# AIML-IfI/openset-imagenet

Hardware: AMD Instinct MI355X
Metric: images/sec (whole node) ResNet-50 + entropic-open-set, Protocol 2, 1/2/4/8 GPUs (higher is better)
Workload: dtype f32; 1 GPU; Protocol 2, ResNet-50, entropic open-set loss, batch 128/GPU; workload_key=p2, classes=30, batch_per_gpu=128, global_batch=128, image=3x224x224, loss=entropic, optimizer=adam lr=1e-3, parallelism=dp1

## Files before the change

openset-imagenet_amd/csrc/conv_wino.hip:

```cpp
#include "conv_common.h"
#include <algorithm>
#include <type_traits>
#include <utility>

using namespace osi_conv;

namespace {

#ifndef OSI_WABL
#define OSI_WABL 0
#endif
#ifndef OSI_FABL
#define OSI_FABL 0
#endif
#ifndef OSI_STAGE_OUT
#define OSI_STAGE_OUT 1
#endif
#ifndef OSI_XSPREAD
#define OSI_XSPREAD 8
#endif
constexpr int KC = 16;
constexpr int PF = 6;

struct WinoP {
// ... 236 lines not shown
#pragma unroll
        for (int j = 0; j < 2; ++j) {
            const int yy = 2 * th + i, xx = 2 * tw + j;
            const bool ok = live && t < p.T && yy < p.H && xx < p.W;
            po[i * 2 + j] = ok ? (uint32_t)((((b * p.H + yy) * p.W + xx) * p.Nc + (WIDE ? 128 : 64) * nt + 32 * wm + 4 * hh) * 4) : OOB;
        }
}

template <bool XF, int EPI, bool ODD, bool WIDE>
__global__ __launch_bounds__(256, 1) void k_wino(WinoP p) {
    constexpr int TB = WIDE ? 32 : 64, CW = WIDE ? 128 : 64, NV = WIDE ? 2 : 4;
    __shared__ __attribute__((aligned(16))) float sV[2 * 16 * TB * KC + (WIDE ? 16384 : 0)];
    __shared__ uint32_t sPo[256];
    const int tid = threadIdx.x, lane = tid & 63, wave = tid >> 6, wm = WIDE ? wave : wave >> 1, wn = WIDE ? 0 : wave & 1;
    const __amdgpu_buffer_rsrc_t rx = make_rsrc(p.x, p.x_bytes);
    const __amdgpu_buffer_rsrc_t ry = make_rsrc(p.y, p.y_bytes);
    const __amdgpu_buffer_rsrc_t ru = make_rsrc(p.u, p.u_bytes);
    const int G = gridDim.x, wg = blockIdx.x;
    const int ltile = WIDE ? tid >> 3 : tid >> 2, q = WIDE ? tid & 7 : tid & 3;
    const int ntile = 32 * wn + (lane & 31), hh = lane >> 5;
    const int THW = p.TH * p.TW;

    Seg seg = seg_first(wg, p.nfull, p.q, p.r, p.KS, G);
    if (!seg.valid) return;
    int mt, nt;
    unit_of(seg.v, p.MT, p.NT, mt, nt);

    uint32_t off[16];
    unsigned long long okm[16];
    uint32_t po[4], po_next[4];
    uint32_t ua, ua_next;
    auto setup = [&](int mt_, int nt_, bool live, uint32_t (&po_)[4], uint32_t& ua_) {
        {
            const int t = mt_ * TB + ltile;
            const int b = t / THW, rem = t - b * THW, th = rem / p.TW, tw = rem - th * p.TW;
            const uint32_t base = (uint32_t)((((b * p.H + 2 * th - 1) * p.W + 2 * tw - 1) * p.Kc + q * NV) * 4);
#pragma unroll
            for (int i = 0; i < 4; ++i)
#pragma unroll
                for (int j = 0; j < 4; ++j) {
                    const int yy = 2 * th - 1 + i, xx = 2 * tw - 1 + j;
                    const bool ok = live && t < p.T && (unsigned)yy < (unsigned)p.H && (unsigned)xx < (unsigned)p.W;
                    off[i * 4 + j] = ok ? base + (uint32_t)((i * p.W + j) * p.Kc * 4) : OOB;
                    if constexpr (XF) okm[i * 4 + j] = __builtin_amdgcn_ballot_w64(ok);
                }
        }
        out_offsets<WIDE>(p, mt_, nt_, ntile, wm, hh, live, po_);
        ua_ = (uint32_t)((((CW / 32) * nt_ + wm) * 2 * 64 + lane) * 16);
    };
    setup(mt, nt, true, po, ua);
    float* const wbase = sV + ltile * KC + (WIDE ? 4 * ((q >> 1) ^ ((ltile >> 2) & 3)) + 2 * (q & 1) : 4 * (q ^ ((ltile >> 2) & 3)));
    const float* const rb0 = sV + ntile * KC + 4 * ((0 + hh) ^ ((ntile >> 2) & 3));
    const float* const rb1 = sV + ntile * KC + 4 * ((2 + hh) ^ ((ntile >> 2) & 3));
    const uint32_t ustep = (uint32_t)p.CB * 2048;

    f32x16 acc[16];
    using XT = std::conditional_t<WIDE, f32x2, f32x4>;
    XT xr[16];
    auto load_x1 = [&](int ks, int k) {
        if constexpr (WIDE) xr[k] = __builtin_bit_cast(f32x2, __builtin_amdgcn_raw_buffer_load_b64(rx, off[k], (uint32_t)ks * (KC * 4), 0));
        else xr[k] = bld4(rx, off[k], (uint32_t)ks * (KC * 4));
    };
    auto load_x = [&](int ks) {
#pragma unroll
        for (int k = 0; k < 16; ++k) load_x1(ks, k);
    };
    auto act_col = [&](int j, const f32x4& sc4, const f32x4& sh4) {
        if constexpr (XF) {
#pragma unroll
            for (int i = 0; i < 4; ++i)
#pragma unroll
                for (int e = 0; e < NV; ++e)
                    asm volatile("v_fma_f32 %0, %0, %1, %2\n\tv_max_f32 %0, 0, %0\n\tv_cndmask_b32 %0, 0, %0, %3"
                                 : "+v"(xr[i * 4 + j][e]) : "v"(sc4[e]), "v"(sh4[e]), "s"(okm[i * 4 + j]));
        }
        {
            const XT d0 = xr[j], d1 = xr[4 + j], d2 = xr[8 + j], d3 = xr[12 + j];
            xr[j] = pk_sub(d0, d2); xr[4 + j] = pk_add(d1, d2); xr[8 + j] = pk_sub(d2, d1); xr[12 + j] = pk_sub(d1, d3);
        }
    };
    auto row_store = [&](int i, int buf) {
        float* w = wbase + buf * (16 * TB * KC) + (i * 4) * (TB * KC);
        const XT t0 = xr[i * 4], t1 = xr[i * 4 + 1], t2 = xr[i * 4 + 2], t3 = xr[i * 4 + 3];
        const XT o[4] = {pk_sub(t0, t2), pk_add(t1, t2), pk_sub(t2, t1), pk_sub(t1, t3)};
#pragma unroll
        for (int nu = 0; nu < 4; ++nu) *reinterpret_cast<XT*>(w + nu * (TB * KC)) = o[nu];
    };
    auto ld_scale = [&](int ks, f32x4& sc4, f32x4& sh4) {
        if constexpr (XF) {
            if constexpr (WIDE) {
                const f32x2 a = *reinterpret_cast<const f32x2*>(p.sc + ks * KC + 2 * q), b = *reinterpret_cast<const f32x2*>(p.sh + ks * KC + 2 * q);
                sc4[0] = a[0]; sc4[1] = a[1]; sh4[0] = b[0]; sh4[1] = b[1];
            } else {
                sc4 = ld4(p.sc + ks * KC + 4 * q);
                sh4 = ld4(p.sh + ks * KC + 4 * q);
            }
        }
    };

    f32x4 sc4 = {1, 1, 1, 1}, sh4 = {0, 0, 0, 0};
    load_x(seg.ks0);
    ld_scale(seg.ks0, sc4, sh4);
#pragma unroll
    for (int j = 0; j < 4; ++j) act_col(j, sc4, sh4);
#pragma unroll
    for (int i = 0; i < 4; ++i) row_store(i, 0);

    f32x4 a[16][2];
    auto load_u = [&](int pos, uint32_t base, int ks) {
        const uint32_t soff = (OSI_FABL & 1) ? 0u : (uint32_t)(pos * p.KS + ks) * ustep;
        a[pos][0] = bld4(ru, base, soff);
        a[pos][1] = bld4(ru, base + 1024u, soff);
    };
#pragma unroll
    for (int i = 0; i < PF; ++i) load_u(i, ua, seg.ks0);
    __syncthreads();

    int buf = 0;
    for (;;) {
#pragma unroll
        for (int i = 0; i < 16; ++i)
#pragma unroll
            for (int r = 0; r < 16; ++r) acc[i][r] = 0.f;
        Seg nxt{0, 0, 0, -1, false};
        const int cur_mt = mt, cur_nt = nt;
        for (int ks = seg.ks0; ks < seg.ks1; ++ks) {
            const bool last = ks + 1 == seg.ks1;
            int ksn = ks + 1;
            uint32_t uan = ua;
            if (last) {
                nxt = seg_next(seg, wg, p.nfull, p.q, p.r, p.KS, G);
                if (nxt.valid) unit_of(nxt.v, p.MT, p.NT, mt, nt);
                setup(mt, nt, nxt.valid, po_next, ua_next);
                ksn = nxt.valid ? nxt.ks0 : 0;
                uan = nxt.valid ? ua_next : ua;
            }
#if !(OSI_FABL & 2) && !OSI_XSPREAD
            load_x(ksn);
#endif
            ld_scale(ksn, sc4, sh4);
            const float* r0 = rb0 + buf * (16 * TB * KC);
            const float* r1 = rb1 + buf * (16 * TB * KC);
            f32x4 b0 = *reinterpret_cast<const f32x4*>(r0), b1 = *reinterpret_cast<const f32x4*>(r1);
            __builtin_amdgcn_sched_barrier(0);
            auto position = [&](auto POSC) {
                constexpr int pos = decltype(POSC)::value;
                if (pos + PF < 16) load_u(pos + PF, ua, ks);
                else load_u(pos + PF - 16, uan, ksn);
#if OSI_XSPREAD && !(OSI_FABL & 2)
                if constexpr (pos < OSI_XSPREAD) {
                    constexpr int n0 = pos * 16 / OSI_XSPREAD, n1 = (pos + 1) * 16 / OSI_XSPREAD;
#pragma unroll
                    for (int k = n0; k < n1; ++k) load_x1(ksn, k);
                }
#endif
                f32x4 nb0 = b0, nb1 = b1;
                if (pos < 15 && !(OSI_FABL & 8)) {
                    nb0 = *reinterpret_cast<const f32x4*>(r0 + (pos + 1) * (TB * KC));
                    nb1 = *reinterpret_cast<const f32x4*>(r1 + (pos + 1) * (TB * KC));
                }
                const f32x4 a0 = a[pos][0], a1 = a[pos][1];
#pragma unroll
                for (int e = 0; e < 4; ++e) acc[pos] = __builtin_amdgcn_mfma_f32_32x32x2f32(a0[e], b0[e], acc[pos], 0, 0, 0);
#pragma unroll
                for (int e = 0; e < 4; ++e) acc[pos] = __builtin_amdgcn_mfma_f32_32x32x2f32(a1[e], b1[e], acc[pos], 0, 0, 0);
#if !(OSI_FABL & 4)
                if constexpr (pos >= 8 && pos < 12) act_col(pos - 8, sc4, sh4);
                if constexpr (pos >= 12) row_store(pos - 12, buf ^ 1);
#endif
                b0 = nb0; b1 = nb1;
                __builtin_amdgcn_sched_barrier(0);
            };
            for_each_const(position, std::make_integer_sequence<int, 16>{});
            __syncthreads();
            buf ^= 1;
        }

        const int ch0 = CW * cur_nt + 32 * wm + 4 * hh;
        const int part = cur_mt * (TB / 16) + 2 * wn + ((lane >> 4) & 1);
        const __amdgpu_buffer_rsrc_t rs = make_rsrc(p.slab, p.slab_bytes);
        const __amdgpu_buffer_rsrc_t r0y = make_rsrc(EPI == 1 ? p.ey0 : p.y, p.y_bytes);
        Epi1Ops L1{};
        if constexpr (EPI == 1) { if (seg.slot < 0) L1 = epi1_load(p, r0y, 0, po, ch0); }
        float* const stage = WIDE ? sV + 2 * 16 * TB * KC : sV + (buf ^ 1) * (16 * TB * KC);
        if (seg.slot < 0 && wm == 0 && hh == 0) {
#pragma unroll
            for (int k = 0; k < 4; ++k) sPo[ntile * 4 + k] = po[k];
        }
#pragma unroll
        for (int g = (OSI_FABL & 16) ? 3 : 0; g < 4; ++g) {
            f32x4 o[4];
#pragma unroll
            for (int e = 0; e < 4; ++e) {
                const int r = 4 * g + e;
                float s[2][4];
#pragma unroll
                for (int nu = 0; nu < 4; ++nu) {
                    float m0, m1, m2, m3;
                    asm volatile("v_accvgpr_read_b32 %0, %1" : "=v"(m0) : "a"(acc[nu][r]));
                    asm volatile("v_accvgpr_read_b32 %0, %1" : "=v"(m1) : "a"(acc[4 + nu][r]));
                    asm volatile("v_accvgpr_read_b32 %0, %1" : "=v"(m2) : "a"(acc[8 + nu][r]));
                    asm volatile("v_accvgpr_read_b32 %0, %1" : "=v"(m3) : "a"(acc[12 + nu][r]));
                    s[0][nu] = m0 + m1 + m2;
                    s[1][nu] = m1 - m2 - m3;
                }
#pragma unroll
                for (int i = 0; i < 2; ++i) {
                    o[i * 2][e] = s[i][0] + s[i][1] + s[i][2];
                    o[i * 2 + 1][e] = s[i][1] - s[i][2] - s[i][3];
                }
            }
            if (seg.slot < 0) {
                auto put = [&](int k, int gq, const f32x4& v) {
#if OSI_STAGE_OUT
                    const int chunk = (32 * wm + 8 * gq + 4 * hh) >> 2;
                    *reinterpret_cast<f32x4*>(stage + (ntile * 4 + k) * CW + 4 * (chunk ^ (ntile & 15))) = v;
#else
                    bst4(ry, v, po[k] == OOB ? OOB : po[k] + 32u * gq, 0);
#endif
                };
                if constexpr (EPI == 0) epi0_quad<ODD>(p, put, g, o, po, ch0, part, lane);
                else if constexpr (EPI == 2) epi2_quad(p, put, g, o, ld4(p.osc + ch0 + 8 * g), ld4(p.osh + ch0 + 8 * g));
                else {
                    const Epi1Ops Ln = epi1_load(p, r0y, g < 3 ? g + 1 : 3, po, ch0);
                    epi1_apply<ODD>(p, put, g, o, po, ch0, part, lane, L1);
                    L1 = Ln;
                }
            } else {
                const uint32_t so = (uint32_t)((wg * 2 + seg.slot) * 65536 + ((wave * 4 + g) * 4) * 1024 + lane * 16);
#pragma unroll
                for (int k = 0; k < 4; ++k) bst4(rs, o[k], so + (uint32_t)k * 1024u, 0);
            }
        }
        if (OSI_STAGE_OUT && seg.slot < 0) {
            __syncthreads();
            constexpr int CPR = CW / 4, NCH = TB * 4 * CPR;
#pragma unroll 4
            for (int it = 0; it < NCH / 256; ++it) {
                const int idx = it * 256 + tid, row = idx / CPR, chunk = idx % CPR;
                const f32x4 v = *reinterpret_cast<const f32x4*>(stage + row * CW + 4 * (chunk ^ ((row >> 2) & 15)));
                const uint32_t base = sPo[row];
                bst4(ry, v, base == OOB ? OOB : base + (uint32_t)chunk * 16u, 0);
            }
            __syncthreads();
        }
        if (!nxt.valid) break;
        seg = nxt;
#pragma unroll
        for (int k = 0; k < 4; ++k) po[k] = po_next[k];
        ua = ua_next;
    }
}

template <int EPI, bool ODD, bool WIDE>
__global__ __launch_bounds__(64) void k_wino_fixup(WinoP p, int G) {
    const int lane = threadIdx.x, u = blockIdx.x >> 4, wave = (blockIdx.x >> 2) & 3, g = blockIdx.x & 3;
    const int wm = WIDE ? wave : wave >> 1, wn = WIDE ? 0 : wave & 1;
    const int ntile = 32 * wn + (lane & 31), hh = lane >> 5;
    int mt, nt;
    unit_of(p.q * G + u, p.MT, p.NT, mt, nt);
    uint32_t po[4];
    out_offsets<WIDE>(p, mt, nt, ntile, wm, hh, true, po);
    const __amdgpu_buffer_rsrc_t ry = make_rsrc(p.y, p.y_bytes);
    const __amdgpu_buffer_rsrc_t rs = make_rsrc(p.slab, p.slab_bytes);
    const int s0 = u * p.KS, s1 = s0 + p.KS;
    int w = (int)(((long)s0 * G) / ((long)p.r * p.KS));
    w = w > 0 ? w - 1 : 0;
    while (piece_begin(w + 1, p.r, p.KS, G) <= s0) ++w;
    f32x4 o[4] = {{0.f, 0.f, 0.f, 0.f}, {0.f, 0.f, 0.f, 0.f}, {0.f, 0.f, 0.f, 0.f}, {0.f, 0.f, 0.f, 0.f}};
    int b0 = piece_begin(w, p.r, p.KS, G);
    for (int ww = w; ww < G && b0 < s1; ++ww) {
        const int b1 = piece_begin(ww + 1, p.r, p.KS, G);
        if (b1 > b0) {
            const int slot = (b0 / p.KS == u) ? 0 : 1;
            const uint32_t so = (uint32_t)((ww * 2 + slot) * 65536 + ((wave * 4 + g) * 4) * 1024 + lane * 16);
#pragma unroll
            for (int k = 0; k < 4; ++k) o[k] += bld4(rs, so + (uint32_t)k * 1024u, 0);
        }
        b0 = b1;
    }
    const int ch0 = (WIDE ? 128 : 64) * nt + 32 * wm + 4 * hh, part = mt * (WIDE ? 2 : 4) + 2 * wn + ((lane >> 4) & 1);
    auto put = [&](int k, int gq, const f32x4& v) { bst4(ry, v, po[k] == OOB ? OOB : po[k] + 32u * gq, 0); };
    if constexpr (EPI == 0) epi0_quad<ODD>(p, put, g, o, po, ch0, part, lane);
    else if constexpr (EPI == 2) epi2_quad(p, put, g, o, ld4(p.osc + ch0 + 8 * g), ld4(p.osh + ch0 + 8 * g));
    else {
        const Epi1Ops L = epi1_load(p, make_rsrc(p.ey0, p.y_bytes), g, po, ch0);
        epi1_apply<ODD>(p, put, g, o, po, ch0, part, lane, L);
    }
}

struct WgradP {
    const float* x;
    const float* dy;
    float* slab;
    const float* sc;
    const float* sh;
    int H, W, Cin, Cout, TH, TW, T;
    int CBn, S, steps;
    int x_bytes, dy_bytes;
    FastDiv dTHW, dTW;
};

template <bool XF>
__global__ __launch_bounds__(256, 1) void k_wino_wgrad(WgradP p) {
    __shared__ __attribute__((aligned(16))) float sL[2 * 2 * 16 * 2 * 64 * 4];
    const int tid = threadIdx.x, lane = tid & 63, wave = tid >> 6, wm = wave >> 1, wn = wave & 1;
    const int item = blockIdx.x;
    const int split = item % p.S, blk = item / p.S, cb = blk % p.CBn, kb = blk / p.CBn;
    const int lh = __builtin_amdgcn_readfirstlane(wave & 1), kkp = __builtin_amdgcn_readfirstlane(wave >> 1);
    const uint32_t xlane = (uint32_t)((cb * 64 + lane) * 4), dlane = (uint32_t)((kb * 64 + lane) * 4);
    const int t_first = split * p.steps * 8;
    const __amdgpu_buffer_rsrc_t rx = make_rsrc(p.x, p.x_bytes);
    const __amdgpu_buffer_rsrc_t rd = make_rsrc(p.dy, p.dy_bytes);
    f32x2 scsh = {1.f, 0.f};
    if constexpr (XF) { scsh[0] = p.sc[cb * 64 + lane]; scsh[1] = p.sh[cb * 64 + lane]; }
    const int cin4 = p.Cin * 4, cout4 = p.Cout * 4;

    f32x2 rx_[2][16], rd_[2][4];
    unsigned okx_[2][2], okd_[2][2];
    uint32_t srb[2][4], scb[2][4], sdr[2][2], sdc[2][2];
    auto prep_step = [&](int st, auto SETC) {
        constexpr int set = decltype(SETC)::value;
#pragma unroll
        for (int i2 = 0; i2 < 2; ++i2) {
            const int tl = 4 * kkp + 2 * i2 + lh;
            const int t_raw = __builtin_amdgcn_readfirstlane(t_first + st * 8 + tl);
            const bool live = t_raw < p.T;
            const uint32_t t = (uint32_t)(live ? t_raw : p.T - 1);
            const uint32_t b = fdiv(t, p.dTHW), rem = t - b * p.dTHW.d, th = fdiv(rem, p.dTW), tw = rem - th * p.dTW.d;
            const int y0 = 2 * (int)th - 1, x0 = 2 * (int)tw - 1;
            unsigned rok = 0, cok = 0;
#pragma unroll
            for (int i = 0; i < 4; ++i) {
                const int yy = y0 + i, xx = x0 + i;
                rok |= ((unsigned)yy < (unsigned)p.H) ? (1u << i) : 0u;
                cok |= ((unsigned)xx < (unsigned)p.W) ? (1u << i) : 0u;
                srb[i2][i] = (uint32_t)((((int)b * p.H + min(max(yy, 0), p.H - 1)) * p.W) * cin4);
                scb[i2][i] = (uint32_t)(min(max(xx, 0), p.W - 1) * cin4);
            }
            if (!live) rok = 0;
            unsigned ok = 0;
#pragma unroll
            for (int i = 0; i < 4; ++i) ok |= ((rok >> i) & 1u) ? (cok << (4 * i)) : 0u;
            okx_[set][i2] = ok;
#pragma unroll
            for (int i = 0; i < 2; ++i) {
                sdr[i2][i] = (uint32_t)(((int)b * p.H + min(y0 + 1 + i, p.H - 1)) * p.W) * (uint32_t)cout4;
                sdc[i2][i] = (uint32_t)min(x0 + 1 + i, p.W - 1) * (uint32_t)cout4;
            }
            okd_[set][i2] = (((rok >> 1) & 1u) ? ((cok >> 1) & 3u) : 0u) | (((rok >> 2) & 1u) ? (((cok >> 1) & 3u) << 2) : 0u);
        }
    };
    auto issue_load = [&](auto NC, auto SETC) {
        constexpr int n = decltype(NC)::value, set = decltype(SETC)::value, i2 = n / 20, k = n % 20;
        if constexpr (k < 16)
            rx_[set][k][i2] = __builtin_bit_cast(float, __builtin_amdgcn_raw_buffer_load_b32(rx, xlane, srb[i2][k / 4] + scb[i2][k % 4], 0));
        else
            rd_[set][k - 16][i2] = __builtin_bit_cast(float, __builtin_amdgcn_raw_buffer_load_b32(rd, dlane, sdr[i2][(k - 16) / 2] + sdc[i2][(k - 16) % 2], 0));
    };
    auto load_step = [&](int st, auto SETC) {
        prep_step(st, SETC);
        auto one = [&](auto NC) { issue_load(NC, SETC); };
        for_each_const(one, std::make_integer_sequence<int, 40>{});
    };
    auto img = [&](int buf, int op, int pos, int h, int ch) { return sL + ((((buf * 2 + op) * 16 + pos) * 2 + h) * 64 + ch) * 4; };
    auto act = [&](auto SETC) {
        constexpr int set = decltype(SETC)::value;
#pragma unroll
        for (int k = 0; k < 16; ++k) {
            f32x2 v = rx_[set][k];
            if constexpr (XF) {
                asm volatile("v_pk_fma_f32 %0, %0, %1, %1 op_sel:[0,0,1] op_sel_hi:[1,0,1]" : "+v"(v) : "v"(scsh));
                asm volatile("v_max_f32 %0, 0, %0" : "+v"(v[0]));
                asm volatile("v_max_f32 %0, 0, %0" : "+v"(v[1]));
            }
            v[0] = ((okx_[set][0] >> k) & 1u) ? v[0] : 0.f;
            v[1] = ((okx_[set][1] >> k) & 1u) ? v[1] : 0.f;
            rx_[set][k] = v;
        }
#pragma unroll
        for (int k = 0; k < 4; ++k) {
            rd_[set][k][0] = ((okd_[set][0] >> k) & 1u) ? rd_[set][k][0] : 0.f;
            rd_[set][k][1] = ((okd_[set][1] >> k) & 1u) ? rd_[set][k][1] : 0.f;
        }
    };
    auto col_x = [&](auto SETC) {
        constexpr int set = decltype(SETC)::value;
#pragma unroll
        for (int j = 0; j < 4; ++j) {
            const f32x2 d0 = rx_[set][j], d1 = rx_[set][4 + j], d2 = rx_[set][8 + j], d3 = rx_[set][12 + j];
            rx_[set][j] = pk_sub(d0, d2); rx_[set][4 + j] = pk_add(d1, d2); rx_[set][8 + j] = pk_sub(d2, d1); rx_[set][12 + j] = pk_sub(d1, d3);
        }
    };
    auto row_store = [&](auto SETC, int i, int buf) {
        constexpr int set = decltype(SETC)::value;
        const f32x2 t0 = rx_[set][i * 4], t1 = rx_[set][i * 4 + 1], t2 = rx_[set][i * 4 + 2], t3 = rx_[set][i * 4 + 3];
        const f32x2 v[4] = {pk_sub(t0, t2), pk_add(t1, t2), pk_sub(t2, t1), pk_sub(t1, t3)};
        const f32x2 a = rd_[set][0], b = rd_[set][1], c = rd_[set][2], d = rd_[set][3];
        const f32x2 e0 = i == 0 ? a : i == 1 ? pk_add(a, c) : i == 2 ? pk_sub(a, c) : pk_neg(c);
        const f32x2 e1 = i == 0 ? b : i == 1 ? pk_add(b, d) : i == 2 ? pk_sub(b, d) : pk_neg(d);
        const f32x2 y[4] = {e0, pk_add(e0, e1), pk_sub(e0, e1), pk_neg(e1)};
#pragma unroll
        for (int nu = 0; nu < 4; ++nu) {
            *reinterpret_cast<f32x2*>(img(buf, 1, i * 4 + nu, lh, lane) + 2 * kkp) = v[nu];
            *reinterpret_cast<f32x2*>(img(buf, 0, i * 4 + nu, lh, lane) + 2 * kkp) = y[nu];
        }
    };

    f32x16 acc[16];
#pragma unroll
    for (int i = 0; i < 16; ++i)
#pragma unroll
        for (int r = 0; r < 16; ++r) acc[i][r] = 0.f;

    using S0 = std::integral_constant<int, 0>;
    using S1 = std::integral_constant<int, 1>;
    load_step(0, S0{});
    load_step(p.steps > 1 ? 1 : 0, S1{});
    act(S0{}); col_x(S0{});
#pragma unroll
    for (int i = 0; i < 4; ++i) row_store(S0{}, i, 0);
    __syncthreads();

    const int hh = lane >> 5, l31 = lane & 31;
    constexpr int TR0 = 10;
    for (int st = 0; st < p.steps; ++st) {
        const int buf = st & 1;
        {
#pragma unroll
            for (int k = 0; k < 16; ++k) rx_[0][k] = rx_[1][k];
#pragma unroll
            for (int k = 0; k < 4; ++k) rd_[0][k] = rd_[1][k];
#pragma unroll
            for (int i2 = 0; i2 < 2; ++i2) { okx_[0][i2] = okx_[1][i2]; okd_[0][i2] = okd_[1][i2]; }
        }
#if !(OSI_WABL & 1)
        prep_step(st + 2 < p.steps ? st + 2 : p.steps - 1, S1{});
#endif
        const float* ra = img(buf, 0, 0, hh, 32 * wm + l31);
        const float* rb = img(buf, 1, 0, hh, 32 * wn + l31);
        f32x4 a0 = *reinterpret_cast<const f32x4*>(ra), b0 = *reinterpret_cast<const f32x4*>(rb);
        __builtin_amdgcn_sched_barrier(0);
        auto position = [&](auto POSC) {
            constexpr int pos = decltype(POSC)::value;
            f32x4 na = a0, nb = b0;
            if (pos < 15) {
                na = *reinterpret_cast<const f32x4*>(ra + (pos + 1) * (2 * 64 * 4));
                nb = *reinterpret_cast<const f32x4*>(rb + (pos + 1) * (2 * 64 * 4));
            }
#pragma unroll
            for (int e = 0; e < 4; ++e) acc[pos] = __builtin_amdgcn_mfma_f32_32x32x2f32(a0[e], b0[e], acc[pos], 0, 0, 0);
#if !(OSI_WABL & 1)
            {
                constexpr int n0 = pos * 40 / 16, n1 = (pos + 1) * 40 / 16;
                if constexpr (n1 > n0) issue_load(std::integral_constant<int, n0>{}, S1{});
                if constexpr (n1 > n0 + 1) issue_load(std::integral_constant<int, n0 + 1>{}, S1{});
                if constexpr (n1 > n0 + 2) issue_load(std::integral_constant<int, n0 + 2>{}, S1{});
            }
#endif
#if !(OSI_WABL & 2)
            if constexpr (pos == TR0) act(S0{});
            if constexpr (pos == TR0 + 1) col_x(S0{});
            if constexpr (pos >= 12) row_store(S0{}, pos - 12, buf ^ 1);
#endif
            a0 = na; b0 = nb;
            __builtin_amdgcn_sched_barrier(0);
        };
        for_each_const(position, std::make_integer_sequence<int, 16>{});
        __syncthreads();
    }

    int lane_e;
    asm volatile("v_mbcnt_lo_u32_b32 %0, -1, 0\n\tv_mbcnt_hi_u32_b32 %0, -1, %0" : "=v"(lane_e));
    const int hh_e = lane_e >> 5, l31_e = lane_e & 31;
    float* out = p.slab + (size_t)item * (9 * 4096) + (32 * lh + l31_e);
#pragma unroll
    for (int r = 0; r < 16; ++r) {
        const int m = 32 * kkp + (r & 3) + 8 * (r >> 2) + 4 * hh_e;
        float t[3][4];
#pragma unroll
        for (int nu = 0; nu < 4; ++nu) {
            const float s0 = acc[nu][r], s1 = acc[4 + nu][r], s2 = acc[8 + nu][r], s3 = acc[12 + nu][r];
            t[0][nu] = s0 + 0.5f * (s1 + s2);
            t[1][nu] = 0.5f * (s1 - s2);
            t[2][nu] = 0.5f * (s1 + s2) + s3;
        }
#pragma unroll
        for (int rr = 0; rr < 3; ++rr) {
            out[(size_t)((rr * 3 + 0) * 64 + m) * 64] = t[rr][0] + 0.5f * (t[rr][1] + t[rr][2]);
            out[(size_t)((rr * 3 + 1) * 64 + m) * 64] = 0.5f * (t[rr][1] - t[rr][2]);
            out[(size_t)((rr * 3 + 2) * 64 + m) * 64] = 0.5f * (t[rr][1] + t[rr][2]) + t[rr][3];
        }
    }
}

__global__ __launch_bounds__(256) void k_wino_wgrad_reduce(const float* __restrict__ slab, float* __restrict__ dw, int Cin, int Cout, int CBn, int S,
                                                           int SG) {
    __shared__ f32x4 part[256];
    const int per = 256 / SG;
    const int o = threadIdx.x % per, g = threadIdx.x / per;
    const int idx = blockIdx.x * per + o;
    const int C4 = Cin / 4, n = Cout * 9 * C4;
    f32x4 a = {0.f, 0.f, 0.f, 0.f};
    int k = 0, tap = 0, c4 = 0;
    if (idx < n) {
        c4 = idx % C4; tap = (idx / C4) % 9; k = idx / (C4 * 9);
        const int cb = (c4 * 4) / 64, kb = k / 64;
        const float* src = slab + (size_t)((kb * CBn + cb) * S) * (9 * 4096) + (size_t)(tap * 64 + (k & 63)) * 64 + ((c4 * 4) & 63);
        for (int s = g; s < S; s += SG) a += ld4(src + (size_t)s * (9 * 4096));
    }
    part[threadIdx.x] = a;
    __syncthreads();
    if (g == 0 && idx < n) {
        for (int j = 1; j < SG; ++j) a += part[j * per + o];
        *reinterpret_cast<f32x4*>(dw + ((size_t)k * 9 + tap) * Cin + c4 * 4) = a;
    }
}

int backward_exclusive_cus();
struct WgradPlan { int S, steps; size_t slab_floats; };
WgradPlan plan_wgrad_wino(const osi_conv_desc* d) {
    const int T = d->B * ((d->H + 1) / 2) * ((d->W + 1) / 2);
    const int blocks = (d->Cout / 64) * (d->Cin / 64);
    int G = backward_exclusive_cus();
    int S = G / blocks;
    if (S < 1) S = 1;
    const int max_s = (T + 63) / 64;
    if (S > max_s) S = max_s;
    const int per = (T + S - 1) / S;
    WgradPlan w;
    w.S = S; w.steps = (per + 7) / 8;
    w.slab_floats = (size_t)blocks * S * 9 * 4096;
    return w;
}

bool wino_shape(const osi_conv_desc* d) {
    return conv_desc_ok(d) && d->R == 3 && d->S == 3 && d->stride == 1 && d->pad == 1 && d->H == d->Ho && d->W == d->Wo && d->H >= 2 && d->W >= 2;
}

struct Geo { int TH, TW, T, MT, P; bool odd; float cnt; bool uniform; };
Geo geo_of(const osi_conv_desc* d) {
    Geo g{};
    g.TH = (d->H + 1) / 2; g.TW = (d->W + 1) / 2; g.T = d->B * g.TH * g.TW; g.MT = (g.T + 63) / 64; g.P = (g.T + 15) / 16;
    const bool even = d->H % 2 == 0 && d->W % 2 == 0;
    g.odd = !even || g.T % 64 != 0;
    const int thw = g.TH * g.TW;
    if (g.P == 1) { g.uniform = true; g.cnt = (float)((long)d->B * d->H * d->W); }
    else if (g.T % 16 == 0 && even) { g.uniform = true; g.cnt = 64.f; }
    else if (g.T % 16 == 0 && 16 % thw == 0) { g.uniform = true; g.cnt = (float)(16 / thw * d->H * d->W); }
    else { g.uniform = false; g.cnt = 64.f; }
    return g;
}

template <int FLIP>
int launch_weights(const float* w, float* u, int Kc, int Nc, hipStream_t st) {
    hipLaunchKernelGGL(k_wino_weights<FLIP>, dim3((unsigned)((Kc / 4 * Nc + 255) / 256)), dim3(256), 0, st, w, u, Kc, Nc, Kc / KC, Nc / 32);
    OSI_LAUNCH_CHECK();
    return OSI_OK;
}

bool wide_units(int Nc) { return g_osi_tuning.wino_wide && Nc % 128 == 0; }

WinoP make_wp(const osi_conv_desc* d, const Geo& g, int Kc, int Nc) {
    WinoP p{};
    const bool wide = wide_units(Nc);
    p.H = d->H; p.W = d->W; p.Kc = Kc; p.Nc = Nc; p.TH = g.TH; p.TW = g.TW; p.T = g.T; p.KS = Kc / KC; p.CB = Nc / 32;
    p.MT = wide ? (g.T + 31) / 32 : g.MT; p.NT = Nc / (wide ? 128 : 64);
    p.x_bytes = (int)((size_t)d->B * d->H * d->W * Kc * 4);
    p.y_bytes = (int)((size_t)d->B * d->H * d->W * Nc * 4);
    p.u_bytes = (int)((size_t)16 * Kc * Nc * 4);
    p.P = g.P; p.cnt = g.cnt; p.rcnt = 1.f / g.cnt;
    return p;
}

int backward_exclusive_cus() {
    if (g_osi_tuning.tail_cus > 0) return chip_cus();
    int res = 8 * g_osi_tuning.dp_reserved_cus;
    if (res > hw_cus() / 4) res = hw_cus() / 4;
    const int n = hw_cus() - res;
    return n < 8 ? 8 : n;
}
int wino_grid(bool backward) {
    int cus = backward ? backward_exclusive_cus() : chip_cus();
    if (cus > hw_cus()) cus = hw_cus();
    cus = cus / 8 * 8;
    return cus < 8 ? 8 : cus;
}
constexpr size_t SLOT_BYTES = 65536;
size_t u_bytes_of(const osi_conv_desc* d) { return ((size_t)16 * d->Cin * d->Cout * sizeof(float) + 255) / 256 * 256; }
size_t slab_bytes_of() { return (size_t)(hw_cus() / 8 * 8 < 8 ? 8 : hw_cus() / 8 * 8) * 2 * SLOT_BYTES; }

void plan_units(WinoP& p, void* slab, size_t slab_bytes, const osi_conv_desc* d, int G, bool input_gradient) {
    const int V = p.MT * p.NT;
    p.q = V / G; p.r = V - p.q * G; p.nfull = p.q * G;
    const bool heavy_tail = p.r > 0 && (double)(G - p.r) / (double)G / (double)(p.q + 1) >= 0.15;
    const int sk = g_osi_tuning.wino_streamk;
    const bool cut = sk == 1 || (sk == 2 && !input_gradient) || (sk == 3 && input_gradient);
    if (!cut || (p.KS <= 4 && !heavy_tail)) { p.nfull = V; p.r = 0; }
    p.slab = (float*)slab;
    p.slab_bytes = (int)std::min<size_t>(slab_bytes, (size_t)hw_cus() * 2 * SLOT_BYTES);
}

}

extern "C" {

int osi_conv_wino_eligible(const osi_conv_desc* d, int input_gradient) {
    if (!wino_shape(d)) return 0;
    const int Kc = input_gradient ? d->Cout : d->Cin, Nc = input_gradient ? d->Cin : d->Cout;
    if (Kc % KC || Nc % 64) return 0;
    const Geo g = geo_of(d);
    return (input_gradient || g.uniform) ? 1 : 0;
}

size_t osi_conv_wino_workspace(const osi_conv_desc* d) {
    if (!wino_shape(d)) return 0;
    return u_bytes_of(d) + slab_bytes_of();
}

static int fwd_wino_impl(const osi_conv_desc* d, const float* x, const float* in_scale, const float* in_shift, const float* w, float* u,
                         float* y, void* slab, size_t slab_bytes, float* pstats, size_t pstats_bytes, int* P, int* rows_per_block,
                         osi_stream_t stream, const osi_conv_epilogue* epi = nullptr) {
    OSI_REQUIRE(x && u && y && slab && osi_conv_wino_eligible(d, 0));
    OSI_REQUIRE(!epi || (epi->scale && epi->shift && !epi->residual && !in_scale && !pstats));
    OSI_REQUIRE((in_scale == nullptr) == (in_shift == nullptr));
    OSI_REQUIRE(slab_bytes >= slab_bytes_of());
    OSI_REQUIRE(!pstats || (P && rows_per_block));
    hipStream_t st = (hipStream_t)stream;
    const Geo g = geo_of(d);
    WinoP p = make_wp(d, g, d->Cin, d->Cout);
    p.x = x; p.u = u; p.y = y; p.sc = in_scale; p.sh = in_shift;
    if (epi) { p.osc = epi->scale; p.osh = epi->shift; p.orelu = epi->relu ? 1 : 0; }
    if (pstats) {
        OSI_REQUIRE(pstats_bytes >= (size_t)2 * g.P * d->Cout * sizeof(float));
        p.pmean = pstats; p.pm2 = pstats + (size_t)g.P * d->Cout;
        *P = g.P; *rows_per_block = (int)g.cnt;
    }
    if (w) { if (int e = launch_weights<0>(w, u, d->Cin, d->Cout, st)) return e; }
    const int G = wino_grid(false);
    OSI_REQUIRE(slab_bytes >= (size_t)G * 2 * SLOT_BYTES);
    plan_units(p, slab, slab_bytes, d, G, false);
    const dim3 grid((unsigned)G), blk(256);
    const bool wide = wide_units(d->Cout), odd = g.odd || (wide && g.T % 32 != 0);
    auto launch = [&](auto XFC, auto ODDC, auto WIDEC) {
        constexpr bool xf = decltype(XFC)::value, od = decltype(ODDC)::value, wd = decltype(WIDEC)::value;
        hipLaunchKernelGGL((k_wino<xf, 0, od, wd>), grid, blk, 0, st, p);
        if (hipGetLastError() != hipSuccess) return OSI_ERR_LAUNCH;
        if (p.r > 0) {
            hipLaunchKernelGGL((k_wino_fixup<0, od, wd>), dim3((unsigned)p.r * 16), dim3(64), 0, st, p, G);
            if (hipGetLastError() != hipSuccess) return OSI_ERR_LAUNCH;
        }
        return OSI_OK;
    };
    auto launch_epi = [&](auto ODDC, auto WIDEC) {
        constexpr bool od = decltype(ODDC)::value, wd = decltype(WIDEC)::value;
        hipLaunchKernelGGL((k_wino<false, 2, od, wd>), grid, blk, 0, st, p);
        if (hipGetLastError() != hipSuccess) return OSI_ERR_LAUNCH;
        if (p.r > 0) {
            hipLaunchKernelGGL((k_wino_fixup<2, od, wd>), dim3((unsigned)p.r * 16), dim3(64), 0, st, p, G);
            if (hipGetLastError() != hipSuccess) return OSI_ERR_LAUNCH;
        }
        return OSI_OK;
    };
    using T_ = std::true_type; using F_ = std::false_type;
    if (epi) {
        if (odd) return wide ? launch_epi(T_{}, T_{}) : launch_epi(T_{}, F_{});
        return wide ? launch_epi(F_{}, T_{}) : launch_epi(F_{}, F_{});
    }
    const int sel = (in_scale ? 4 : 0) | (odd ? 2 : 0) | (wide ? 1 : 0);
    switch (sel) {
        case 0: return launch(F_{}, F_{}, F_{});
        case 1: return launch(F_{}, F_{}, T_{});
        case 2: return launch(F_{}, T_{}, F_{});
        case 3: return launch(F_{}, T_{}, T_{});
        case 4: return launch(T_{}, F_{}, F_{});
        case 5: return launch(T_{}, F_{}, T_{});
        case 6: return launch(T_{}, T_{}, F_{});
        default: return launch(T_{}, T_{}, T_{});
    }
}

int osi_conv_fwd_wino(const osi_conv_desc* d, const float* x, const float* in_scale, const float* in_shift, const float* w, float* y,
                      void* ws, size_t ws_bytes, float* pstats, size_t pstats_bytes, int* P, int* rows_per_block, osi_stream_t stream) {
    OSI_REQUIRE(w && ws && wino_shape(d) && ws_bytes >= osi_conv_wino_workspace(d));
    return fwd_wino_impl(d, x, in_scale, in_shift, w, (float*)ws, y, (char*)ws + u_bytes_of(d), ws_bytes - u_bytes_of(d), pstats, pstats_bytes, P,
                         rows_per_block, stream);
}

size_t osi_conv_wino_weights_bytes(const osi_conv_desc* d) { return wino_shape(d) ? u_bytes_of(d) : 0; }
size_t osi_conv_wino_slab_bytes(void) { return slab_bytes_of(); }
int osi_conv_wino_transform_weights(const osi_conv_desc* d, const float* w, int input_gradient, float* u, size_t u_bytes, osi_stream_t stream) {
    OSI_REQUIRE(w && u && osi_conv_wino_eligible(d, input_gradient ? 1 : 0) && u_bytes >= u_bytes_of(d));
    return input_gradient ? launch_weights<1>(w, u, d->Cout, d->Cin, (hipStream_t)stream) : launch_weights<0>(w, u, d->Cin, d->Cout, (hipStream_t)stream);
}
int osi_conv_fwd_wino_pre(const osi_conv_desc* d, const float* x, const float* in_scale, const float* in_shift, const float* u, float* y,
                          void* slab, size_t slab_bytes, float* pstats, size_t pstats_bytes, int* P, int* rows_per_block, osi_stream_t stream) {
    return fwd_wino_impl(d, x, in_scale, in_shift, nullptr, const_cast<float*>(u), y, slab, slab_bytes, pstats, pstats_bytes, P, rows_per_block, stream);
}

int osi_conv_fwd_wino_epilogue_pre(const osi_conv_desc* d, const float* x, const float* u, float* out, const osi_conv_epilogue* e, void* slab,
                                   size_t slab_bytes, osi_stream_t stream) {
    OSI_REQUIRE(e);
    return fwd_wino_impl(d, x, nullptr, nullptr, nullptr, const_cast<float*>(u), out, slab, slab_bytes, nullptr, 0, nullptr, nullptr, stream, e);
}

static int dgrad_wino_impl(const osi_conv_desc* d, const float* dy, const float* w, float* u, float* dx, const osi_dgrad_fusion* f, void* slab,
                           size_t slab_bytes, int* P, osi_stream_t stream) {
    OSI_REQUIRE(dy && u && dx && slab && f && P && osi_conv_wino_eligible(d, 1));
    OSI_REQUIRE(!f->relu_mask && !f->y1 && !f->pool_idx && f->addend_stride != 2);
    OSI_REQUIRE(f->y0 && f->scale0 && f->shift0);
    OSI_REQUIRE(!f->partials || (f->mean0 && f->invstd0));
    OSI_REQUIRE(slab_bytes >= slab_bytes_of());
    hipStream_t st = (hipStream_t)stream;
    const Geo g = geo_of(d);
    WinoP p = make_wp(d, g, d->Cout, d->Cin);
    p.x = dy; p.u = u; p.y = dx;
    p.ey0 = f->y0; p.escale0 = f->scale0; p.eshift0 = f->shift0;
    p.emean0 = f->mean0 ? f->mean0 : f->scale0; p.einv0 = f->invstd0 ? f->invstd0 : f->scale0;
    if (f->partials) {
        OSI_REQUIRE(f->partials_bytes >= (size_t)3 * g.P * d->Cin * sizeof(float));
        p.esum = f->partials;
    }
    *P = g.P;
    if (w) { if (int e = launch_weights<1>(w, u, d->Cout, d->Cin, st)) return e; }
    const int G = wino_grid(true);
    OSI_REQUIRE(slab_bytes >= (size_t)G * 2 * SLOT_BYTES);
    plan_units(p, slab, slab_bytes, d, G, true);
    const dim3 grid((unsigned)G), blk(256);
    const bool wide = wide_units(d->Cin), odd = g.odd || (wide && g.T % 32 != 0);
    auto launch = [&](auto ODDC, auto WIDEC) {
        constexpr bool od = decltype(ODDC)::value, wd = decltype(WIDEC)::value;
        hipLaunchKernelGGL((k_wino<false, 1, od, wd>), grid, blk, 0, st, p);
        if (hipGetLastError() != hipSuccess) return OSI_ERR_LAUNCH;
        if (p.r > 0) {
            hipLaunchKernelGGL((k_wino_fixup<1, od, wd>), dim3((unsigned)p.r * 16), dim3(64), 0, st, p, G);
            if (hipGetLastError() != hipSuccess) return OSI_ERR_LAUNCH;
        }
        return OSI_OK;
    };
    using T_ = std::true_type; using F_ = std::false_type;
    if (odd) return wide ? launch(T_{}, T_{}) : launch(T_{}, F_{});
    return wide ? launch(F_{}, T_{}) : launch(F_{}, F_{});
}

int osi_conv_dgrad_fused_wino(const osi_conv_desc* d, const float* dy, const float* w, float* dx, const osi_dgrad_fusion* f, void* ws,
                              size_t ws_bytes, int* P, osi_stream_t stream) {
    OSI_REQUIRE(w && ws && wino_shape(d) && ws_bytes >= osi_conv_wino_workspace(d));
    return dgrad_wino_impl(d, dy, w, (float*)ws, dx, f, (char*)ws + u_bytes_of(d), ws_bytes - u_bytes_of(d), P, stream);
}
int osi_conv_dgrad_fused_wino_pre(const osi_conv_desc* d, const float* dy, const float* u, float* dx, const osi_dgrad_fusion* f, void* slab,
                                  size_t slab_bytes, int* P, osi_stream_t stream) {
    return dgrad_wino_impl(d, dy, nullptr, const_cast<float*>(u), dx, f, slab, slab_bytes, P, stream);
}

size_t osi_conv_wgrad_wino_workspace(const osi_conv_desc* d) {
    if (!wino_shape(d) || d->Cin % 64 || d->Cout % 64) return 0;
    return plan_wgrad_wino(d).slab_floats * sizeof(float);
}

int osi_conv_wgrad_wino(const osi_conv_desc* d, const float* dy, const float* x, const float* in_scale, const float* in_shift, float* dw,
                        void* ws, size_t ws_bytes, osi_stream_t stream) {
    OSI_REQUIRE(dy && x && dw && ws && wino_shape(d) && d->Cin % 64 == 0 && d->Cout % 64 == 0);
    OSI_REQUIRE((in_scale == nullptr) == (in_shift == nullptr));
    const WgradPlan w = plan_wgrad_wino(d);
    OSI_REQUIRE(ws_bytes >= w.slab_floats * sizeof(float));
    hipStream_t st = (hipStream_t)stream;
    WgradP p{};
    p.x = x; p.dy = dy; p.slab = (float*)ws; p.sc = in_scale; p.sh = in_shift;
    p.H = d->H; p.W = d->W; p.Cin = d->Cin; p.Cout = d->Cout; p.TH = (d->H + 1) / 2; p.TW = (d->W + 1) / 2; p.T = d->B * p.TH * p.TW;
    p.CBn = d->Cin / 64; p.S = w.S; p.steps = w.steps;
    p.dTHW = make_fastdiv((uint32_t)(p.TH * p.TW)); p.dTW = make_fastdiv((uint32_t)p.TW);
    p.x_bytes = (int)((size_t)d->B * d->H * d->W * d->Cin * 4);
    p.dy_bytes = (int)((size_t)d->B * d->H * d->W * d->Cout * 4);
    const dim3 grid((unsigned)((d->Cout / 64) * p.CBn * p.S)), blk(256);
    if (in_scale) hipLaunchKernelGGL((k_wino_wgrad<true>), grid, blk, 0, st, p);
    else hipLaunchKernelGGL((k_wino_wgrad<false>), grid, blk, 0, st, p);
    OSI_LAUNCH_CHECK();
    const int n = d->Cout * 9 * (d->Cin / 4);
    int SG = 1;
    while (SG * 2 <= p.S && SG < 16) SG *= 2;
    const int per = 256 / SG;
    hipLaunchKernelGGL(k_wino_wgrad_reduce, dim3((unsigned)((n + per - 1) / per)), blk, 0, st, (const float*)ws, dw, d->Cin, d->Cout, p.CBn, p.S, SG);
    OSI_LAUNCH_CHECK();
    return OSI_OK;
}

}
```

Baseline: 4405 images/sec.

## Split Winograd wgrad positions across 8 waves with LDS epilogue exchange

The Winograd weight-gradient kernel now runs 512 threads instead of 256. Each wave handles one tile per step instead of two, and the 16 transform positions are split into two halves of 8 owned by different wave groups. This halves the accumulator registers per wave (8 MFMA accumulators instead of 16) so more waves can hide memory latency. Prefetch is deepened to three steps, with loads and transforms interleaved across the 8-position loop. The output transform now needs an LDS exchange between paired waves, and the wider workgroup costs extra sync and possible LDS contention.

```diff
diff --git a/openset-imagenet_amd/csrc/conv_wino.hip b/openset-imagenet_amd/csrc/conv_wino.hip
--- a/openset-imagenet_amd/csrc/conv_wino.hip
+++ b/openset-imagenet_amd/csrc/conv_wino.hip
@@ -562,196 +562,207 @@
 };
 
 template <bool XF>
-__global__ __launch_bounds__(256, 1) void k_wino_wgrad(WgradP p) {
+__global__ __launch_bounds__(512) void k_wino_wgrad(WgradP p) {
     __shared__ __attribute__((aligned(16))) float sL[2 * 2 * 16 * 2 * 64 * 4];
-    const int tid = threadIdx.x, lane = tid & 63, wave = tid >> 6, wm = wave >> 1, wn = wave & 1;
+    const int tid = threadIdx.x, lane = tid & 63, hh = lane >> 5, l31 = lane & 31;
+    const int wave = __builtin_amdgcn_readfirstlane(tid >> 6);
+    const int ph = wave >> 2, wm = (wave >> 1) & 1, wn = wave & 1;
     const int item = blockIdx.x;
     const int split = item % p.S, blk = item / p.S, cb = blk % p.CBn, kb = blk / p.CBn;
-    const int lh = __builtin_amdgcn_readfirstlane(wave & 1), kkp = __builtin_amdgcn_readfirstlane(wave >> 1);
+    const int lh = wave & 1, kq = wave >> 1;
     const uint32_t xlane = (uint32_t)((cb * 64 + lane) * 4), dlane = (uint32_t)((kb * 64 + lane) * 4);
     const int t_first = split * p.steps * 8;
     const __amdgpu_buffer_rsrc_t rx = make_rsrc(p.x, p.x_bytes);
     const __amdgpu_buffer_rsrc_t rd = make_rsrc(p.dy, p.dy_bytes);
-    f32x2 scsh = {1.f, 0.f};
-    if constexpr (XF) { scsh[0] = p.sc[cb * 64 + lane]; scsh[1] = p.sh[cb * 64 + lane]; }
+    float sc = 1.f, sh = 0.f;
+    if constexpr (XF) { sc = p.sc[cb * 64 + lane]; sh = p.sh[cb * 64 + lane]; }
     const int cin4 = p.Cin * 4, cout4 = p.Cout * 4;
 
-    f32x2 rx_[2][16], rd_[2][4];
-    unsigned okx_[2][2], okd_[2][2];
-    uint32_t srb[2][4], scb[2][4], sdr[2][2], sdc[2][2];
+    float rx_[2][16], rd_[2][4];
+    unsigned okx_[2], okd_[2];
+    uint32_t srb[4], scb[4], sdr[2], sdc[2];
     auto prep_step = [&](int st, auto SETC) {
         constexpr int set = decltype(SETC)::value;
-#pragma unroll
-        for (int i2 = 0; i2 < 2; ++i2) {
-            const int tl = 4 * kkp + 2 * i2 + lh;
-            const int t_raw = __builtin_amdgcn_readfirstlane(t_first + st * 8 + tl);
-            const bool live = t_raw < p.T;
-            const uint32_t t = (uint32_t)(live ? t_raw : p.T - 1);
-            const uint32_t b = fdiv(t, p.dTHW), rem = t - b * p.dTHW.d, th = fdiv(rem, p.dTW), tw = rem - th * p.dTW.d;
-            const int y0 = 2 * (int)th - 1, x0 = 2 * (int)tw - 1;
-            unsigned rok = 0, cok = 0;
-#pragma unroll
-            for (int i = 0; i < 4; ++i) {
-                const int yy = y0 + i, xx = x0 + i;
-                rok |= ((unsigned)yy < (unsigned)p.H) ? (1u << i) : 0u;
-                cok |= ((unsigned)xx < (unsigned)p.W) ? (1u << i) : 0u;
-                srb[i2][i] = (uint32_t)((((int)b * p.H + min(max(yy, 0), p.H - 1)) * p.W) * cin4);
-                scb[i2][i] = (uint32_t)(min(max(xx, 0), p.W - 1) * cin4);
-            }
-            if (!live) rok = 0;
-            unsigned ok = 0;
-#pragma unroll
-            for (int i = 0; i < 4; ++i) ok |= ((rok >> i) & 1u) ? (cok << (4 * i)) : 0u;
-            okx_[set][i2] = ok;
-#pragma unroll
-            for (int i = 0; i < 2; ++i) {
-                sdr[i2][i] = (uint32_t)(((int)b * p.H + min(y0 + 1 + i, p.H - 1)) * p.W) * (uint32_t)cout4;
-                sdc[i2][i] = (uint32_t)min(x0 + 1 + i, p.W - 1) * (uint32_t)cout4;
-            }
-            okd_[set][i2] = (((rok >> 1) & 1u) ? ((cok >> 1) & 3u) : 0u) | (((rok >> 2) & 1u) ? (((cok >> 1) & 3u) << 2) : 0u);
-        }
+        const int t_raw = t_first + st * 8 + wave;
+        const bool live = t_raw < p.T;
+        const uint32_t t = (uint32_t)(live ? t_raw : p.T - 1);
+        const uint32_t b = fdiv(t, p.dTHW), rem = t - b * p.dTHW.d, th = fdiv(rem, p.dTW), tw = rem - th * p.dTW.d;
+        const int y0 = 2 * (int)th - 1, x0 = 2 * (int)tw - 1;
+        unsigned rok = 0, cok = 0;
+#pragma unroll
+        for (int i = 0; i < 4; ++i) {
+            const int yy = y0 + i, xx = x0 + i;
+            rok |= ((unsigned)yy < (unsigned)p.H) ? (1u << i) : 0u;
+            cok |= ((unsigned)xx < (unsigned)p.W) ? (1u << i) : 0u;
+            srb[i] = (uint32_t)((((int)b * p.H + min(max(yy, 0), p.H - 1)) * p.W) * cin4);
+            scb[i] = (uint32_t)(min(max(xx, 0), p.W - 1) * cin4);
+        }
+        if (!live) rok = 0;
+        unsigned ok = 0;
+#pragma unroll
+        for (int i = 0; i < 4; ++i) ok |= ((rok >> i) & 1u) ? (cok << (4 * i)) : 0u;
+        okx_[set] = ok;
+#pragma unroll
+        for (int i = 0; i < 2; ++i) {
+            sdr[i] = (uint32_t)(((int)b * p.H + min(y0 + 1 + i, p.H - 1)) * p.W) * (uint32_t)cout4;
+            sdc[i] = (uint32_t)min(x0 + 1 + i, p.W - 1) * (uint32_t)cout4;
+        }
+        okd_[set] = (((rok >> 1) & 1u) ? ((cok >> 1) & 3u) : 0u) | (((rok >> 2) & 1u) ? (((cok >> 1) & 3u) << 2) : 0u);
     };
     auto issue_load = [&](auto NC, auto SETC) {
-        constexpr int n = decltype(NC)::value, set = decltype(SETC)::value, i2 = n / 20, k = n % 20;
-        if constexpr (k < 16)
-            rx_[set][k][i2] = __builtin_bit_cast(float, __builtin_amdgcn_raw_buffer_load_b32(rx, xlane, srb[i2][k / 4] + scb[i2][k % 4], 0));
+        constexpr int n = decltype(NC)::value, set = decltype(SETC)::value;
+        if constexpr (n < 16)
+            rx_[set][n] = __builtin_bit_cast(float, __builtin_amdgcn_raw_buffer_load_b32(rx, xlane, srb[n / 4] + scb[n % 4], 0));
         else
-            rd_[set][k - 16][i2] = __builtin_bit_cast(float, __builtin_amdgcn_raw_buffer_load_b32(rd, dlane, sdr[i2][(k - 16) / 2] + sdc[i2][(k - 16) % 2], 0));
+            rd_[set][n - 16] = __builtin_bit_cast(float, __builtin_amdgcn_raw_buffer_load_b32(rd, dlane, sdr[(n - 16) / 2] + sdc[(n - 16) % 2], 0));
     };
     auto load_step = [&](int st, auto SETC) {
         prep_step(st, SETC);
         auto one = [&](auto NC) { issue_load(NC, SETC); };
-        for_each_const(one, std::make_integer_sequence<int, 40>{});
+        for_each_const(one, std::make_integer_sequence<int, 20>{});
     };
     auto img = [&](int buf, int op, int pos, int h, int ch) { return sL + ((((buf * 2 + op) * 16 + pos) * 2 + h) * 64 + ch) * 4; };
+    float tx[16], td[4];
     auto act = [&](auto SETC) {
         constexpr int set = decltype(SETC)::value;
 #pragma unroll
         for (int k = 0; k < 16; ++k) {
-            f32x2 v = rx_[set][k];
-            if constexpr (XF) {
-                asm volatile("v_pk_fma_f32 %0, %0, %1, %1 op_sel:[0,0,1] op_sel_hi:[1,0,1]" : "+v"(v) : "v"(scsh));
-                asm volatile("v_max_f32 %0, 0, %0" : "+v"(v[0]));
-                asm volatile("v_max_f32 %0, 0, %0" : "+v"(v[1]));
-            }
-            v[0] = ((okx_[set][0] >> k) & 1u) ? v[0] : 0.f;
-            v[1] = ((okx_[set][1] >> k) & 1u) ? v[1] : 0.f;
-            rx_[set][k] = v;
-        }
-#pragma unroll
-        for (int k = 0; k < 4; ++k) {
-            rd_[set][k][0] = ((okd_[set][0] >> k) & 1u) ? rd_[set][k][0] : 0.f;
-            rd_[set][k][1] = ((okd_[set][1] >> k) & 1u) ? rd_[set][k][1] : 0.f;
-        }
-    };
-    auto col_x = [&](auto SETC) {
-        constexpr int set = decltype(SETC)::value;
+            float v = rx_[set][k];
+            if constexpr (XF) asm volatile("v_fma_f32 %0, %1, %2, %3\n\tv_max_f32 %0, 0, %0" : "=v"(v) : "v"(rx_[set][k]), "v"(sc), "v"(sh));
+            tx[k] = ((okx_[set] >> k) & 1u) ? v : 0.f;
+        }
+#pragma unroll
+        for (int k = 0; k < 4; ++k) td[k] = ((okd_[set] >> k) & 1u) ? rd_[set][k] : 0.f;
+    };
+    auto col_x = [&]() {
 #pragma unroll
         for (int j = 0; j < 4; ++j) {
-            const f32x2 d0 = rx_[set][j], d1 = rx_[set][4 + j], d2 = rx_[set][8 + j], d3 = rx_[set][12 + j];
-            rx_[set][j] = pk_sub(d0, d2); rx_[set][4 + j] = pk_add(d1, d2); rx_[set][8 + j] = pk_sub(d2, d1); rx_[set][12 + j] = pk_sub(d1, d3);
-        }
-    };
-    auto row_store = [&](auto SETC, int i, int buf) {
-        constexpr int set = decltype(SETC)::value;
-        const f32x2 t0 = rx_[set][i * 4], t1 = rx_[set][i * 4 + 1], t2 = rx_[set][i * 4 + 2], t3 = rx_[set][i * 4 + 3];
-        const f32x2 v[4] = {pk_sub(t0, t2), pk_add(t1, t2), pk_sub(t2, t1), pk_sub(t1, t3)};
-        const f32x2 a = rd_[set][0], b = rd_[set][1], c = rd_[set][2], d = rd_[set][3];
-        const f32x2 e0 = i == 0 ? a : i == 1 ? pk_add(a, c) : i == 2 ? pk_sub(a, c) : pk_neg(c);
-        const f32x2 e1 = i == 0 ? b : i == 1 ? pk_add(b, d) : i == 2 ? pk_sub(b, d) : pk_neg(d);
-        const f32x2 y[4] = {e0, pk_add(e0, e1), pk_sub(e0, e1), pk_neg(e1)};
+            const float d0 = tx[j], d1 = tx[4 + j], d2 = tx[8 + j], d3 = tx[12 + j];
+            tx[j] = d0 - d2; tx[4 + j] = d1 + d2; tx[8 + j] = d2 - d1; tx[12 + j] = d1 - d3;
+        }
+    };
+    auto row_store = [&](int i, int buf) {
+        const float t0 = tx[i * 4], t1 = tx[i * 4 + 1], t2 = tx[i * 4 + 2], t3 = tx[i * 4 + 3];
+        const float v[4] = {t0 - t2, t1 + t2, t2 - t1, t1 - t3};
+        const float a = td[0], b = td[1], c = td[2], d = td[3];
+        const float e0 = i == 0 ? a : i == 1 ? a + c : i == 2 ? a - c : 0.f - c;
+        const float e1 = i == 0 ? b : i == 1 ? b + d : i == 2 ? b - d : 0.f - d;
+        const float y[4] = {e0, e0 + e1, e0 - e1, 0.f - e1};
 #pragma unroll
         for (int nu = 0; nu < 4; ++nu) {
-            *reinterpret_cast<f32x2*>(img(buf, 1, i * 4 + nu, lh, lane) + 2 * kkp) = v[nu];
-            *reinterpret_cast<f32x2*>(img(buf, 0, i * 4 + nu, lh, lane) + 2 * kkp) = y[nu];
-        }
-    };
-
-    f32x16 acc[16];
-#pragma unroll
-    for (int i = 0; i < 16; ++i)
+            img(buf, 1, i * 4 + nu, lh, lane)[kq] = v[nu];
+            img(buf, 0, i * 4 + nu, lh, lane)[kq] = y[nu];
+        }
+    };
+
+    f32x16 acc[8];
+#pragma unroll
+    for (int i = 0; i < 8; ++i)
 #pragma unroll
         for (int r = 0; r < 16; ++r) acc[i][r] = 0.f;
 
     using S0 = std::integral_constant<int, 0>;
     using S1 = std::integral_constant<int, 1>;
+    const int last = p.steps - 1;
     load_step(0, S0{});
-    load_step(p.steps > 1 ? 1 : 0, S1{});
-    act(S0{}); col_x(S0{});
-#pragma unroll
-    for (int i = 0; i < 4; ++i) row_store(S0{}, i, 0);
+    load_step(min(1, last), S1{});
+    __builtin_amdgcn_sched_barrier(0);
+    act(S0{});
+    __builtin_amdgcn_sched_barrier(0);
+    load_step(min(2, last), S0{});
+    __builtin_amdgcn_sched_barrier(0);
+    col_x();
+#pragma unroll
+    for (int i = 0; i < 4; ++i) row_store(i, 0);
     __syncthreads();
 
-    const int hh = lane >> 5, l31 = lane & 31;
-    constexpr int TR0 = 10;
-    for (int st = 0; st < p.steps; ++st) {
-        const int buf = st & 1;
-        {
-#pragma unroll
-            for (int k = 0; k < 16; ++k) rx_[0][k] = rx_[1][k];
-#pragma unroll
-            for (int k = 0; k < 4; ++k) rd_[0][k] = rd_[1][k];
-#pragma unroll
-            for (int i2 = 0; i2 < 2; ++i2) { okx_[0][i2] = okx_[1][i2]; okd_[0][i2] = okd_[1][i2]; }
-        }
-#if !(OSI_WABL & 1)
-        prep_step(st + 2 < p.steps ? st + 2 : p.steps - 1, S1{});
-#endif
-        const float* ra = img(buf, 0, 0, hh, 32 * wm + l31);
-        const float* rb = img(buf, 1, 0, hh, 32 * wn + l31);
+    auto step = [&](int st, auto BUFC) {
+        constexpr int buf = decltype(BUFC)::value;
+        using SET = std::integral_constant<int, 1 - buf>;
+        const float* ra = img(buf, 0, 8 * ph, hh, 32 * wm + l31);
+        const float* rb = img(buf, 1, 8 * ph, hh, 32 * wn + l31);
         f32x4 a0 = *reinterpret_cast<const f32x4*>(ra), b0 = *reinterpret_cast<const f32x4*>(rb);
         __builtin_amdgcn_sched_barrier(0);
         auto position = [&](auto POSC) {
-            constexpr int pos = decltype(POSC)::value;
+            constexpr int lp = decltype(POSC)::value;
             f32x4 na = a0, nb = b0;
-            if (pos < 15) {
-                na = *reinterpret_cast<const f32x4*>(ra + (pos + 1) * (2 * 64 * 4));
-                nb = *reinterpret_cast<const f32x4*>(rb + (pos + 1) * (2 * 64 * 4));
-            }
-#pragma unroll
-            for (int e = 0; e < 4; ++e) acc[pos] = __builtin_amdgcn_mfma_f32_32x32x2f32(a0[e], b0[e], acc[pos], 0, 0, 0);
+            if (lp < 7) {
+                na = *reinterpret_cast<const f32x4*>(ra + (lp + 1) * (2 * 64 * 4));
+                nb = *reinterpret_cast<const f32x4*>(rb + (lp + 1) * (2 * 64 * 4));
+            }
+#pragma unroll
+            for (int e = 0; e < 4; ++e) acc[lp] = __builtin_amdgcn_mfma_f32_32x32x2f32(a0[e], b0[e], acc[lp], 0, 0, 0);
+#if !(OSI_WABL & 2)
+            if constexpr (lp == 0) act(SET{});
+            if constexpr (lp == 1) col_x();
+            if constexpr (lp >= 2 && lp < 6) row_store(lp - 2, buf ^ 1);
+#endif
 #if !(OSI_WABL & 1)
-            {
-                constexpr int n0 = pos * 40 / 16, n1 = (pos + 1) * 40 / 16;
-                if constexpr (n1 > n0) issue_load(std::integral_constant<int, n0>{}, S1{});
-                if constexpr (n1 > n0 + 1) issue_load(std::integral_constant<int, n0 + 1>{}, S1{});
-                if constexpr (n1 > n0 + 2) issue_load(std::integral_constant<int, n0 + 2>{}, S1{});
-            }
-#endif
-#if !(OSI_WABL & 2)
-            if constexpr (pos == TR0) act(S0{});
-            if constexpr (pos == TR0 + 1) col_x(S0{});
-            if constexpr (pos >= 12) row_store(S0{}, pos - 12, buf ^ 1);
+            if constexpr (lp == 0) prep_step(min(st + 3, last), SET{});
+            if constexpr (lp >= 1 && lp <= 7) {
+                constexpr int n0 = (lp - 1) * 20 / 7, n1 = lp * 20 / 7;
+                auto one = [&](auto IC) { issue_load(std::integral_constant<int, n0 + decltype(IC)::value>{}, SET{}); };
+                for_each_const(one, std::make_integer_sequence<int, n1 - n0>{});
+            }
 #endif
             a0 = na; b0 = nb;
             __builtin_amdgcn_sched_barrier(0);
         };
-        for_each_const(position, std::make_integer_sequence<int, 16>{});
+        for_each_const(position, std::make_integer_sequence<int, 8>{});
         __syncthreads();
-    }
-
-    int lane_e;
-    asm volatile("v_mbcnt_lo_u32_b32 %0, -1, 0\n\tv_mbcnt_hi_u32_b32 %0, -1, %0" : "=v"(lane_e));
-    const int hh_e = lane_e >> 5, l31_e = lane_e & 31;
-    float* out = p.slab + (size_t)item * (9 * 4096) + (32 * lh + l31_e);
-#pragma unroll
-    for (int r = 0; r < 16; ++r) {
-        const int m = 32 * kkp + (r & 3) + 8 * (r >> 2) + 4 * hh_e;
-        float t[3][4];
-#pragma unroll
-        for (int nu = 0; nu < 4; ++nu) {
-            const float s0 = acc[nu][r], s1 = acc[4 + nu][r], s2 = acc[8 + nu][r], s3 = acc[12 + nu][r];
-            t[0][nu] = s0 + 0.5f * (s1 + s2);
-            t[1][nu] = 0.5f * (s1 - s2);
-            t[2][nu] = 0.5f * (s1 + s2) + s3;
-        }
-#pragma unroll
-        for (int rr = 0; rr < 3; ++rr) {
-            out[(size_t)((rr * 3 + 0) * 64 + m) * 64] = t[rr][0] + 0.5f * (t[rr][1] + t[rr][2]);
-            out[(size_t)((rr * 3 + 1) * 64 + m) * 64] = 0.5f * (t[rr][1] - t[rr][2]);
-            out[(size_t)((rr * 3 + 2) * 64 + m) * 64] = 0.5f * (t[rr][1] + t[rr][2]) + t[rr][3];
-        }
-    }
+    };
+    for (int st = 0; st < p.steps; st += 2) {
+        step(st, S0{});
+        if (st + 1 < p.steps) step(st + 1, S1{});
+    }
+
+    f32x4* const X = reinterpret_cast<f32x4*>(sL);
+    auto give = [&](auto PHC) {
+        constexpr int PH = decltype(PHC)::value;
+#pragma unroll
+        for (int lp = 0; lp < 8; ++lp)
+#pragma unroll
+            for (int hq = 0; hq < 2; ++hq) {
+                f32x4 v;
+#pragma unroll
+                for (int e = 0; e < 4; ++e) v[e] = acc[lp][8 * (1 - PH) + 4 * hq + e];
+                X[((wave * 8 + lp) * 2 + hq) * 64 + lane] = v;
+            }
+    };
+    if (ph == 0) give(S0{}); else give(S1{});
+    __syncthreads();
+    float* out = p.slab + (size_t)item * (9 * 4096) + (32 * wn + l31);
+    auto finish = [&](auto PHC) {
+        constexpr int PH = decltype(PHC)::value;
+        const f32x4* const Xp = X + ((wave ^ 4) * 16) * 64 + lane;
+#pragma unroll
+        for (int hq = 0; hq < 2; ++hq) {
+            f32x4 o[8];
+#pragma unroll
+            for (int lp = 0; lp < 8; ++lp) o[lp] = Xp[(lp * 2 + hq) * 64];
+#pragma unroll
+            for (int e = 0; e < 4; ++e) {
+                const int r = 8 * PH + 4 * hq + e;
+                const int m = 32 * wm + (r & 3) + 8 * (r >> 2) + 4 * hh;
+                auto S = [&](int pos) { return (pos >> 3) == PH ? acc[pos & 7][r] : o[pos & 7][e]; };
+                float t[3][4];
+#pragma unroll
+                for (int nu = 0; nu < 4; ++nu) {
+                    const float s0 = S(nu), s1 = S(4 + nu), s2 = S(8 + nu), s3 = S(12 + nu);
+                    t[0][nu] = s0 + 0.5f * (s1 + s2);
+                    t[1][nu] = 0.5f * (s1 - s2);
+                    t[2][nu] = 0.5f * (s1 + s2) + s3;
+                }
+#pragma unroll
+                for (int rr = 0; rr < 3; ++rr) {
+                    out[(size_t)((rr * 3 + 0) * 64 + m) * 64] = t[rr][0] + 0.5f * (t[rr][1] + t[rr][2]);
+                    out[(size_t)((rr * 3 + 1) * 64 + m) * 64] = 0.5f * (t[rr][1] - t[rr][2]);
+                    out[(size_t)((rr * 3 + 2) * 64 + m) * 64] = 0.5f * (t[rr][1] + t[rr][2]) + t[rr][3];
+                }
+            }
+        }
+    };
+    if (ph == 0) finish(S0{}); else finish(S1{});
 }
 
 __global__ __launch_bounds__(256) void k_wino_wgrad_reduce(const float* __restrict__ slab, float* __restrict__ dw, int Cin, int Cout, int CBn, int S,
@@ -1033,8 +1044,8 @@
     p.x_bytes = (int)((size_t)d->B * d->H * d->W * d->Cin * 4);
     p.dy_bytes = (int)((size_t)d->B * d->H * d->W * d->Cout * 4);
     const dim3 grid((unsigned)((d->Cout / 64) * p.CBn * p.S)), blk(256);
-    if (in_scale) hipLaunchKernelGGL((k_wino_wgrad<true>), grid, blk, 0, st, p);
-    else hipLaunchKernelGGL((k_wino_wgrad<false>), grid, blk, 0, st, p);
+    if (in_scale) hipLaunchKernelGGL((k_wino_wgrad<true>), grid, dim3(512), 0, st, p);
+    else hipLaunchKernelGGL((k_wino_wgrad<false>), grid, dim3(512), 0, st, p);
     OSI_LAUNCH_CHECK();
     const int n = d->Cout * 9 * (d->Cin / 4);
     int SG = 1;
```

Result: faster. 4457 images/sec (median of 6 runs) (+1.2%).
